# ComputationalPhysiology/oasisx

Measured on AMD Instinct MI355X. Metric: time-steps/sec, 3D Taylor-Green 128^3 P2-P1 (with pressure-CG SpMV GB/s in roofline), higher is better.
Workload: dtype f64

## Files before the change

### include/oasisx_hip.h

```cpp
#ifndef OASISX_HIP_H
#define OASISX_HIP_H

#include <stddef.h>
#include <stdint.h>

#ifdef __cplusplus
extern "C" {
#endif

#define OX_KV 2
#define OX_ROW_BLOCK_WAVES 8
#define OX_ROW_BLOCK_LDS (134 * 1024)
#define OX_SLICE 64

#define OX_CONVERGED_RTOL 2
#define OX_CONVERGED_ATOL 3
#define OX_CONVERGED_ITS 4
#define OX_DIVERGED_ITS (-3)
#define OX_DIVERGED_DTOL (-4)
#define OX_DIVERGED_BREAKDOWN (-5)
#define OX_DIVERGED_NANORINF (-9)

#define OX_KSP_CG 1
#define OX_KSP_BCGS 2
// ... 154 lines not shown
int ox_synchronize(void *stream);

int ox_version(void);
const char *ox_last_error(void);
int ox_sell_kv(void);
int ox_device_info(int *n_cu, char *name, int name_len);

int ox_spmv(const ox_sell *A, const double *x, double *y, int ncomp, const ox_dist *dist,
            void *stream);

int ox_sell_compress_cols(const ox_sell *A, uint16_t *cols16, int32_t *cbase, int64_t *n_compressed,
                          void *stream);

int ox_spmv_multi(int v2s, int gdim, const ox_sell *A, const double *x, const double *base, double scale,
                  double *y, const ox_dist *dist, void *stream);
int ox_assemble_rect(int family, int row_degree, int col_degree, const ox_cells *cells, const ox_adj *adj,
                     const uint8_t *adj_pos, int pw, const ox_sell *A, void *stream);

int ox_axpby(int64_t n, double a, const double *x, double b, const double *y, double *z,
             void *stream);
int ox_dot(int64_t n_rows, int ncomp, const double *x, const double *y, double *out_host,
           const ox_dist *dist, void *stream);

int ox_set_bc(double *b, const int32_t *dofs, const double *g, int64_t n, int ncomp, int comp,
              void *stream);

int ox_scatter_add(double *b, const int32_t *rows, const double *y, int64_t n, int ncomp, int comp,
                   double scale, void *stream);

int ox_zero_rows(const ox_sell *A, const int32_t *rows, int64_t n, double diag, void *stream);
int ox_zero_rows_au(const ox_sell *A, const int32_t *rows, int64_t n, double diag, double *au,
                    const double *u1, int ncomp, void *stream);
int ox_zero_rows_cols(const ox_sell *A, const uint8_t *is_bc, double diag, void *stream);

int ox_assemble_matrix(int kind, int degree, const ox_cells *cells, const int32_t *cell_dofs,
                       const ox_adj *adj, const uint8_t *adj_pos, int pw, const ox_sell *A,
                       int n_bins, const int64_t *bin_ptr_host, const int32_t *bin_slices,
                       const int32_t *bin_width_host, void *stream);
int ox_assemble_weights(int degree, const ox_cells *cells, const ox_adj *adj, int64_t n_rows,
                        double *w, void *stream);
int ox_assemble_load_vector(const ox_cells *cells, const ox_adj *adj, int64_t n_rows, int n_d, int n_q,
                            const double *wphi, const double *fq, double *b, void *stream);

int ox_assemble_first(int degree, const ox_cells *cells, const int32_t *cell_dofs,
                      const ox_adj *adj, const uint8_t *adj_pos, int pw, const ox_sell *A,
                      const ox_sell *M, const ox_sell *K, const double *uab,
// ... 49 lines not shown

size_t ox_ksp_work_bytes(int64_t n_rows, int64_t n_cols, int ncomp, int ksp_type);
int ox_ksp_solve(int ksp_type, const ox_sell *A, const double *dinv, const double *b, double *x,
                 int ncomp, double rtol, double atol, int max_it, int nonzero_guess,
                 int check_every, int max_restarts, void *work, size_t work_bytes,
                 ox_ksp_result *result, const ox_dist *dist, void *stream);
int ox_ksp_solve_ax0(int ksp_type, const ox_sell *A, const double *dinv, const double *b, double *x,
                     int ncomp, double rtol, double atol, int max_it, int nonzero_guess,
                     int check_every, int max_restarts, void *work, size_t work_bytes,
                     ox_ksp_result *result, const ox_dist *dist, void *stream, const double *ax0);
int ox_ksp_solve_dc(int ksp_type, const ox_sell *A, const double *dinv, const double *b, double *x,
                    int ncomp, double rtol, double atol, int max_it, int nonzero_guess,
                    int check_every, int max_restarts, void *work, size_t work_bytes,
                    ox_ksp_result *result, const ox_dist *dist, void *stream, const double *ax0,
                    const uint8_t *dinv_code, const double *dinv_dict, int n_dinv_dict);
typedef struct {
  double rtol, atol, divtol;
  int32_t max_it, nonzero_guess, check_every, max_restarts;
  int32_t fold_blocks, run_ahead;
  const double *ax0;
  const uint8_t *dinv_code;
  const double *dinv_dict;
  int32_t n_dinv_dict;
  int32_t reserved;
} ox_ksp_options;
int ox_ksp_options_default(ox_ksp_options *opt);
int ox_ksp_solve_opt(int ksp_type, const ox_sell *A, const double *dinv, const double *b, double *x, int ncomp,
                     const ox_ksp_options *opt, void *work, size_t work_bytes, ox_ksp_result *result,
                     const ox_dist *dist, void *stream);
size_t ox_ksp_work_bytes_for(const ox_sell *A, int ncomp, int ksp_type);

int ox_dg1_grad_rhs(int u_degree, const ox_cells *cells, const int32_t *cell_dofs, const double *u, double *b,
                    void *stream);
int ox_dg1_mass(int inverse, const ox_cells *cells, int ncomp, const double *in, double *out, void *stream);

int ox_remove_mean(int64_t n, int64_t n_apply, double *x, const double *w, double wsum,
                   const ox_dist *dist, void *stream);

int ox_ksp_default_fold_blocks(void);
int ox_ksp_kernels_per_iteration(int ksp_type, const ox_sell *A, int ncomp, int check_every, int fold_blocks,
                                 int partitioned);
int ox_profile_begin(int max_records, int sample_every);
int ox_profile_end(void);
int ox_profile_get(int tag, long long key, long long *count, double *total_ms);

int ox_range_push(const char *name);
int ox_range_pop(void);
// ... 94 lines not shown
```

### oasisx_amd/_lib.py

```python
from __future__ import annotations

import ctypes as C
import os

_HERE = os.path.dirname(os.path.abspath(__file__))
LIB_PATH = os.environ.get("OX_LIB_PATH") or os.path.join(_HERE, "liboasisx_hip.so")

KSP_CG, KSP_BCGS, KSP_CG_SINGLE, KSP_BCGS_MERGED, KSP_CG_MERGED = 1, 2, 3, 4, 5
KSP_CG_MG = 6
MG_MAX_DEGREE = 8
ROW_BLOCK_WAVES, ROW_BLOCK_LDS = 8, 134 * 1024
CONVERGED_RTOL, CONVERGED_ATOL, CONVERGED_ITS = 2, 3, 4
DIVERGED_ITS, DIVERGED_DTOL, DIVERGED_BREAKDOWN, DIVERGED_NANORINF = -3, -4, -5, -9


class OasisxHipError(RuntimeError):
    pass


class ox_sell(C.Structure):
    _fields_ = [
        ("n_rows", C.c_int64),
        ("n_cols", C.c_int64),
        ("n_slices", C.c_int32),
# ... 144 lines not shown
        ("reason", C.c_int32 * 4),
        ("its", C.c_int32 * 4),
        ("rnorm", C.c_double * 4),
        ("bnorm", C.c_double * 4),
        ("resumed", C.c_int32 * 4),
    ]


class ox_ksp_options(C.Structure):
    _fields_ = [
        ("rtol", C.c_double),
        ("atol", C.c_double),
        ("divtol", C.c_double),
        ("max_it", C.c_int32),
        ("nonzero_guess", C.c_int32),
        ("check_every", C.c_int32),
        ("max_restarts", C.c_int32),
        ("fold_blocks", C.c_int32),
        ("run_ahead", C.c_int32),
        ("ax0", C.c_void_p),
        ("dinv_code", C.c_void_p),
        ("dinv_dict", C.c_void_p),
        ("n_dinv_dict", C.c_int32),
        ("reserved", C.c_int32),
    ]


_P = C.c_void_p
_I = C.c_int
_L = C.c_int64
_D = C.c_double

SIGNATURES = {
    "ox_version": (_I, []),
    "ox_last_error": (C.c_char_p, []),
    "ox_sell_kv": (_I, []),
    "ox_device_info": (_I, [C.POINTER(_I), C.c_char_p, _I]),
    "ox_mesh_create": (_I, [_P, _L, _P, _L, _I, _I, _I, C.POINTER(_P)]),
    "ox_mesh_view": (_I, [_P, C.POINTER(ox_mesh_info)]),
    "ox_mesh_destroy": (_I, [_P]),
    "ox_space_create": (_I, [_P, _I, _I, C.POINTER(_P)]),
    "ox_space_create_ordered": (_I, [_P, _I, _I, _I, C.POINTER(_P)]),
    "ox_mesh_create_sub": (_I, [_P, _L, _P, _L, _I, _I, C.POINTER(_D), C.POINTER(_D), _I, _I, _L, C.POINTER(_P)]),
    "ox_space_create_part": (_I, [_P, _I, _I, _P, _L, _I, _L, C.POINTER(_P)]),
    "ox_space_view": (_I, [_P, C.POINTER(ox_space_info)]),
    "ox_space_windows": (_I, [_P, C.POINTER(ox_window_info)]),
    "ox_space_windows_split": (_I, [_P, _I, C.POINTER(ox_window_info)]),
    "ox_space_destroy": (_I, [_P]),
    "ox_rect_create": (_I, [_P, _P, C.POINTER(_P)]),
    "ox_rect_view": (_I, [_P, C.POINTER(ox_rect_info)]),
    "ox_rect_destroy": (_I, [_P]),
    "ox_value_dictionary": (_I, [_P, _L, _I, _P, _P, C.POINTER(_I), _P]),
    "ox_pair_stream_size": (_I, [C.POINTER(ox_sell), _P, _P, C.POINTER(_L), _P]),
    "ox_pair_stream_fill": (_I, [C.POINTER(ox_sell), _P, _P, _P, _P, C.POINTER(_L), _P]),
    "ox_malloc": (_I, [C.c_size_t, C.POINTER(_P)]),
    "ox_free": (_I, [_P]),
    "ox_memset": (_I, [_P, _I, C.c_size_t, _P]),
    "ox_synchronize": (_I, [_P]),
    "ox_spmv": (_I, [C.POINTER(ox_sell), _P, _P, _I, _P, _P]),
    "ox_sell_compress_cols": (_I, [C.POINTER(ox_sell), _P, _P, C.POINTER(_L), _P]),
    "ox_spmv_multi": (_I, [_I, _I, C.POINTER(ox_sell), _P, _P, _D, _P, _P, _P]),
    "ox_assemble_rect": (_I, [_I, _I, _I, C.POINTER(ox_cells), C.POINTER(ox_adj), _P, _I, C.POINTER(ox_sell), _P]),
    "ox_axpby": (_I, [_L, _D, _P, _D, _P, _P, _P]),
    "ox_dot": (_I, [_L, _I, _P, _P, C.POINTER(_D), _P, _P]),
    "ox_set_bc": (_I, [_P, _P, _P, _L, _I, _I, _P]),
    "ox_scatter_add": (_I, [_P, _P, _P, _L, _I, _I, _D, _P]),
    "ox_zero_rows": (_I, [C.POINTER(ox_sell), _P, _L, _D, _P]),
    "ox_zero_rows_au": (_I, [C.POINTER(ox_sell), _P, _L, _D, _P, _P, _I, _P]),
    "ox_zero_rows_cols": (_I, [C.POINTER(ox_sell), _P, _D, _P]),
    "ox_assemble_matrix": (_I, [_I, _I, C.POINTER(ox_cells), _P, C.POINTER(ox_adj), _P, _I,
                                C.POINTER(ox_sell), _I, C.POINTER(_L), _P, C.POINTER(C.c_int32), _P]),
    "ox_assemble_weights": (_I, [_I, C.POINTER(ox_cells), C.POINTER(ox_adj), _L, _P, _P]),
    "ox_assemble_load_vector": (_I, [C.POINTER(ox_cells), C.POINTER(ox_adj), _L, _I, _I, _P, _P, _P, _P]),
    "ox_assemble_first": (_I, [_I, C.POINTER(ox_cells), _P, C.POINTER(ox_adj), _P, _I,
                               C.POINTER(ox_sell), C.POINTER(ox_sell), C.POINTER(ox_sell), _P, _P, _P, _P, _D,
                               _D, _I, C.POINTER(_L), _P, C.POINTER(C.c_int32), _P]),
    "ox_assemble_first_au": (_I, [_I, C.POINTER(ox_cells), _P, C.POINTER(ox_adj), _P, _I,
                                  C.POINTER(ox_sell), C.POINTER(ox_sell), C.POINTER(ox_sell), _P, _P, _P, _P, _D,
                                  _D, _I, C.POINTER(_L), _P, C.POINTER(C.c_int32), _P, _P]),
    "ox_assemble_matrix_blocks": (_I, [_I, _I, C.POINTER(ox_cells), _P, C.POINTER(ox_adj), _P, _I, C.POINTER(ox_sell), _I, _P,
                                       _L, _P]),
    "ox_assemble_first_blocks": (_I, [_I, C.POINTER(ox_cells), _P, C.POINTER(ox_adj), _P, _I,
                                      C.POINTER(ox_sell), C.POINTER(ox_sell), C.POINTER(ox_sell), _P, _P, _P, _P, _D,
                                      _D, _I, _P, _L, _P, _P]),
    "ox_eddy_viscosity": (_I, [_I, _I, C.POINTER(ox_cells), _P, _P, _D, _P, _P]),
    "ox_assemble_first_au_nut": (_I, [_I, C.POINTER(ox_cells), _P, C.POINTER(ox_adj), _P, _I,
                                      C.POINTER(ox_sell), C.POINTER(ox_sell), C.POINTER(ox_sell), _P, _P, _P, _P, _D,
# ... 123 lines not shown
```

### oasisx_amd/csrc/ox_ksp.hip

```cpp
#include "ox_kernels.h"
#include "ox_ksp_dev.h"
#include "ox_p2p.h"
#include <type_traits>

struct KspPart2 {
  const double *partial;
  int nparts, nv;
};

__device__ __forceinline__ void ksp_gather2(const double *__restrict__ partial, int nparts, int nv, const KspPart2 &B,
                                            double (&v)[OX_MAX_NV]) {
  ox_gather_partials(partial, nparts, nv, v);
  if (B.nv > 0) {
    double w[OX_MAX_NV];
    ox_gather_partials(B.partial, B.nparts, B.nv, w);
#pragma unroll
    for (int i = 0; i < OX_MAX_NV; ++i)
#pragma unroll
      for (int j = 0; j < OX_MAX_NV; ++j)
        if (j == i - nv && j < B.nv) v[i] = w[j];
  }
}


// ... 932 lines not shown
    if (ox_prof_on) ox_prof_stop(st);
    OX_LAUNCH_CHECK();
    return 0;
  }
  hipLaunchKernelGGL((k_ksp_reduce<PH>), dim3(1), dim3(ox_red_threads(nmax)), 0, st, partial, nparts, nv, B, sums);
  OX_LAUNCH_CHECK();
  nv += B.nv;
  if (ox_allreduce_impl(dist, sums, nv, st)) return -1;
  hipLaunchKernelGGL((k_ksp_logic<PH>), dim3(1), dim3(64), 0, st, S, sums, P);
  if (ox_prof_on) ox_prof_stop(st);
  OX_LAUNCH_CHECK();
  return 0;
}

__global__ __launch_bounds__(256) void k_extract_col(int64_t n, const double *__restrict__ src, int nc,
                                                     int c, double *__restrict__ dst) {
  const int64_t stride = (int64_t)gridDim.x * 256;
  for (int64_t i = (int64_t)blockIdx.x * 256 + threadIdx.x; i < n; i += stride) dst[i] = src[i * nc + c];
}
__global__ __launch_bounds__(256) void k_insert_col(int64_t n, const double *__restrict__ src, int nc,
                                                    int c, double *__restrict__ dst) {
  const int64_t stride = (int64_t)gridDim.x * 256;
  for (int64_t i = (int64_t)blockIdx.x * 256 + threadIdx.x; i < n; i += stride) dst[i * nc + c] = src[i];
}

struct KspVecs {
  double *x, *r, *z, *p, *q;
  double *rhat, *v, *s, *t;
  double *u, *w;
};

struct KspCtx {
  const ox_sell *A;
  const double *dinv;
  KspDinv D;
  KspState *S, *S2;
  double *sums, *partial, *partial2;
  const ox_dist *dist;
  hipStream_t st;
  int nb, nbs;
  int fold;
};

#define KSP_SYNC(PH, partial, nparts, nv)                                                       \
  do {                                                                                          \
    if (ksp_sync_point<PH>(C.S, partial, nparts, nv, C.sums, P, C.dist, C.st)) return -1;       \
// ... 350 lines not shown
      if (queue(1 - cur)) return -1;
      it += batch;
    }
    OX_HIP(hipEventSynchronize(g_state_ev[cur]));
    if (C.dist && ox_dist_status(C.dist)) return -1;
    if (g_state_host[1 + cur].done || !more) {
      OX_HIP(hipStreamSynchronize(C.st));
      if (!more && !g_state_host[1 + cur].done) {
        OX_HIP(hipMemcpyAsync(g_state_host, C.S, sizeof(KspState), hipMemcpyDeviceToHost, C.st));
        OX_HIP(hipStreamSynchronize(C.st));
        return 0;
      }
      g_state_host[0] = g_state_host[1 + cur];
      return 0;
    }
    cur = 1 - cur;
  }
}

template <int NC>
static int ksp_run(int ksp_type, const ox_sell *A, const double *dinv, const double *b, double *x,
                   const KspParams &P, int guess, int check_every, char *work,
                   ox_ksp_result *result, const ox_dist *dist, hipStream_t st, const double *ax0, const KspDinv &Dc,
                   int fold_blocks, int run_ahead) {
  const int64_t n = A->n_rows;
  const KspLayout L = ksp_layout(A->n_rows, A->n_cols, NC, ksp_type, ksp_grid_max(A));
  KspCtx C;
  C.A = A;
  C.dinv = dinv;
  C.D = Dc;
  C.S = reinterpret_cast<KspState *>(work + L.state);
  C.S2 = reinterpret_cast<KspState *>(work + L.state2);
  C.sums = reinterpret_cast<double *>(work + L.sums);
  C.partial = reinterpret_cast<double *>(work + L.partial);
  C.partial2 = reinterpret_cast<double *>(work + L.partial2);
  C.dist = dist;
  C.st = st;
  C.nb = ox_vec_blocks(2 * (n > 0 ? n : 1));
  C.nbs = ox_spmv_dist_nparts(A, dist, NC);
  C.fold = fold_blocks;
  double *vec[6];
  for (int i = 0; i < L.nvec; ++i) vec[i] = reinterpret_cast<double *>(work + L.vec0 + L.vec_stride * i);
  if (!g_state_host) OX_HIP(hipHostMalloc(&g_state_host, 3 * sizeof(KspState)));
  const bool cg = ksp_type == OX_KSP_CG, cgs = ksp_type == OX_KSP_CG_SINGLE, bm = ksp_type == OX_KSP_BCGS_MERGED;
  const bool cgm = ksp_type == OX_KSP_CG_MERGED;
  KspVecs V{};
  V.x = x;
// ... 8 lines not shown
    if (ox_spmv_dist(A, V.u, V.w, NC, OX_EPI_DOT, nullptr, nullptr, C.partial2, nullptr, dist, st)) return -1;
    if (ksp_sync_point<PH_CGS_INIT>(C.S, C.partial, C.nb, 3 * NC, C.sums, P, dist, st, KspPart2{C.partial2, C.nbs, NC}))
      return -1;
  } else if (cg || cgm) {
    V.r = vec[0], V.p = vec[1], V.q = vec[2];
    if (guess && !ax0) {
      if (ox_spmv_dist(A, x, V.q, NC, OX_EPI_NONE, nullptr, nullptr, nullptr, nullptr, dist, st)) return -1;
    }
    hipLaunchKernelGGL((k_cg_init<NC>), dim3(C.nb), dim3(256), 0, st, n, b, x, (guess && ax0) ? ax0 : V.q, dinv, V.r,
                       V.p, guess, C.partial);
    OX_LAUNCH_CHECK();
    KSP_SYNC(PH_CG_INIT, C.partial, C.nb, 3 * NC);
  } else {
    V.r = vec[0], V.rhat = vec[1], V.p = vec[2], V.v = vec[3], V.s = vec[4], V.t = vec[5];
    if (guess && !ax0) {
      if (ox_spmv_dist(A, x, V.t, NC, OX_EPI_NONE, nullptr, nullptr, nullptr, nullptr, dist, st)) return -1;
    }
    hipLaunchKernelGGL((k_bcgs_init<NC>), dim3(C.nb), dim3(256), 0, st, n, b, x, (guess && ax0) ? ax0 : V.t, dinv, V.r,
                       V.rhat, V.p, V.v, guess, C.partial);
    OX_LAUNCH_CHECK();
    KSP_SYNC(PH_BCGS_INIT, C.partial, C.nb, 2 * NC);
  }
  bool bm_first = true;
  auto iterate = [&](auto nc_tag, const KspVecs &W, const KspParams &Q) -> int {
    constexpr int N_ = decltype(nc_tag)::value;
    const bool first = bm_first;
    bm_first = false;
    return cgs ? cgs_iterations<N_>(C, W, Q, check_every)
           : cgm ? cgm_iterations<N_>(C, W, Q, check_every, first)
               : (cg ? cg_iterations<N_>(C, W, Q, check_every)
                     : (bm ? bcgsm_iterations<N_>(C, W, Q, check_every, first) : bcgs_iterations<N_>(C, W, Q, check_every, first)));
  };
  auto batch_of = [&](int every) { return every > 8 ? 8 : every; };
  int it = 0;
  bool tail_done = false;
  for (;;) {
    tail_done = false;
    if (NC == 1 && run_ahead) {
      const int bsz = batch_of(check_every);
      auto it1 = [&](int count) -> int {
        const bool first = bm_first;
        bm_first = false;
        return cgs ? cgs_iterations<1>(C, V, P, count)
               : cgm ? cgm_iterations<1>(C, V, P, count, first)
                   : (cg ? cg_iterations<1>(C, V, P, count)
                         : (bm ? bcgsm_iterations<1>(C, V, P, count, first) : bcgs_iterations<1>(C, V, P, count, first)));
      };
      if (ksp_run_ahead(C, it1, bsz, it, P.max_it)) return -1;
    }
    for (; !(NC == 1 && run_ahead) && it <= P.max_it; it += check_every) {
      if (iterate(std::integral_constant<int, NC>{}, V, P)) return -1;
      if (ksp_read_state(C)) return -1;
      if (g_state_host->done) break;
      if (NC > 1) {
        int live = -1, nlive = 0;
        for (int c = 0; c < NC; ++c)
          if (g_state_host->active[c]) live = c, ++nlive;
        if (nlive == 1) {
          double *cv[8];
          for (int i = 0; i < 8; ++i) cv[i] = reinterpret_cast<double *>(work + L.narrow0 + L.narrow_stride * i);
          KspVecs W{};
          double *src[8] = {V.x, V.r, V.z, V.p, V.q, V.rhat, V.v, nullptr};
          double **dst[8] = {&W.x, &W.r, &W.z, &W.p, &W.q, &W.rhat, &W.v, nullptr};
          if (cg) src[2] = nullptr;
          if (cgs) {
            src[2] = V.u, dst[2] = &W.u;
            src[4] = V.s, dst[4] = &W.s;
            src[5] = V.w, dst[5] = &W.w;
            src[6] = nullptr;
          }
          for (int i = 0; i < 7; ++i) {
            *dst[i] = cv[i];
            if (!src[i]) continue;
            hipLaunchKernelGGL(k_extract_col, dim3(C.nb), dim3(256), 0, st, n, src[i], NC, live, cv[i]);
            OX_LAUNCH_CHECK();
          }
          if (!cgs) {
            W.s = cv[2];
            W.t = cv[4];
          }
          KspParams P1 = P;
          P1.nc = 1;
          P1.c0 = live;
          if (run_ahead) {
            const int bsz = batch_of(check_every);
            auto it1 = [&](int count) -> int {
              return cgs ? cgs_iterations<1>(C, W, P1, count)
                         : (cg ? cg_iterations<1>(C, W, P1, count)
                               : (bm ? bcgsm_iterations<1>(C, W, P1, count, false) : bcgs_iterations<1>(C, W, P1, count, false)));
            };
            it += check_every;
            if (ksp_run_ahead(C, it1, bsz, it, P.max_it)) return -1;
          } else {
            for (it += check_every; it <= P.max_it; it += check_every) {
              if (iterate(std::integral_constant<int, 1>{}, W, P1)) return -1;
              if (ksp_read_state(C)) return -1;
              if (g_state_host->done) break;
// ... 188 lines not shown
                               void *work, size_t work_bytes, ox_ksp_result *result, void *stream) {
  if (!mg || !A || !b || !x || !work || !result || !opt) OX_FAIL("ox_ksp_solve_mg: null argument");
  return mgcg_solve(mg, A, b, x, opt, work, work_bytes, result, nullptr, ox_stream(stream));
}

extern "C" int ox_ksp_solve_mg_dist(const ox_mg *mg, const ox_sell *A, const double *b, double *x, const ox_ksp_options *opt,
                                    void *work, size_t work_bytes, ox_ksp_result *result, const ox_dist *dist,
                                    void *stream) {
  if (!A || !b || !x || !work || !result || !opt || !dist) OX_FAIL("ox_ksp_solve_mg_dist: null argument");
  if (!mg && A->n_rows > 0) OX_FAIL("ox_ksp_solve_mg_dist: no hierarchy for %lld owned rows", (long long)A->n_rows);
  return mgcg_solve(mg, A, b, x, opt, work, work_bytes, result, dist, ox_stream(stream));
}

extern "C" int ox_ksp_options_default(ox_ksp_options *o) {
  if (!o) OX_FAIL("ox_ksp_options_default: null argument");
  memset(o, 0, sizeof(*o));
  o->rtol = 1e-5;
  o->atol = 1e-50;
  o->divtol = 1e4;
  o->max_it = 10000;
  o->check_every = 1;
  o->fold_blocks = -1;
  o->run_ahead = -1;
  return 0;
}

extern "C" int ox_ksp_default_fold_blocks(void) { return ksp_fold_blocks_default(); }

extern "C" int ox_ksp_kernels_per_iteration(int ksp_type, const ox_sell *A, int ncomp, int check_every, int fold_blocks,
                                            int partitioned) {
  if (!A) return -1;
  if (ksp_type == OX_KSP_CG_MERGED && ncomp > 1) ksp_type = OX_KSP_CG;
  const bool one = ncomp == 1 && !partitioned && A->n_rows >= 2 && ksp_fold_blocks_of(fold_blocks) > 0;
  const int batch = check_every > 8 ? 8 : (check_every < 1 ? 1 : check_every);
  switch (ksp_type) {
    case OX_KSP_CG: {
      if (!one) return 5;
      return ox_spmv_dist_nparts(A, nullptr, 1) >= OX_PRERED_MIN ? 4 : 3;
    }
    case OX_KSP_CG_MERGED:
      return (one && (batch & 1) == 0 && ox_spmv_dist_nparts(A, nullptr, 1) <= 10 * OX_FOLD_T) ? 2 : 3;
    case OX_KSP_CG_SINGLE: return 3;
    case OX_KSP_BCGS: return 8;
    case OX_KSP_BCGS_MERGED: return 6;
    default: return -1;
  }
// ... 9 lines not shown
  if (ksp_type == OX_KSP_CG_MERGED && ncomp > 1) ksp_type = OX_KSP_CG;
  if (ncomp < 1 || ncomp > OX_MAXC) OX_FAIL("ox_ksp_solve: ncomp=%d out of range", ncomp);
  if (work_bytes < ox_ksp_work_bytes_for(A, ncomp, ksp_type))
    OX_FAIL("ox_ksp_solve: workspace too small (%zu < %zu)", work_bytes, ox_ksp_work_bytes_for(A, ncomp, ksp_type));
  if (opt->dinv_code && (!opt->dinv_dict || opt->n_dinv_dict < 1 || opt->n_dinv_dict > 256))
    OX_FAIL("ox_ksp_solve: dinv dictionary of %d entries", opt->n_dinv_dict);
  if (!(opt->divtol > 0.0)) OX_FAIL("ox_ksp_solve: divtol=%g (must be positive; PETSc's default is 1e4)", opt->divtol);
  const int max_it = opt->max_it < 1 ? 1 : opt->max_it;
  const int check_every = opt->check_every < 1 ? 1 : opt->check_every;
  memset(result, 0, sizeof(*result));
  KspParams P{};
  P.rtol = opt->rtol;
  P.atol = opt->atol;
  P.dtol = opt->divtol;
  P.max_it = max_it;
  P.nc = ncomp;
  P.c0 = 0;
  P.nc_total = ncomp;
  P.max_restarts = opt->max_restarts < 0 ? 0 : opt->max_restarts;
  hipStream_t st = ox_stream(stream);
  char *w = static_cast<char *>(work);
  const KspDinv D{dinv, opt->dinv_code, opt->dinv_dict, opt->dinv_code ? opt->n_dinv_dict : 0};
  const int fold = ksp_fold_blocks_of(opt->fold_blocks), ahead = opt->run_ahead < 0 ? 1 : (opt->run_ahead ? 1 : 0);
  const int guess = opt->nonzero_guess;
  const double *ax0 = opt->ax0;
  switch (ncomp) {
    case 1: return ksp_run<1>(ksp_type, A, dinv, b, x, P, guess, check_every, w, result, dist, st, ax0, D, fold, ahead);
    case 2: return ksp_run<2>(ksp_type, A, dinv, b, x, P, guess, check_every, w, result, dist, st, ax0, D, fold, ahead);
    default: return ksp_run<3>(ksp_type, A, dinv, b, x, P, guess, check_every, w, result, dist, st, ax0, D, fold, ahead);
  }
}

extern "C" int ox_ksp_solve_dc(int ksp_type, const ox_sell *A, const double *dinv, const double *b,
                               double *x, int ncomp, double rtol, double atol, int max_it,
                               int nonzero_guess, int check_every, int max_restarts, void *work,
                               size_t work_bytes, ox_ksp_result *result, const ox_dist *dist, void *stream,
                               const double *ax0, const uint8_t *dinv_code, const double *dinv_dict, int n_dinv_dict) {
  ox_ksp_options o;
  ox_ksp_options_default(&o);
  o.rtol = rtol;
  o.atol = atol;
  o.max_it = max_it;
  o.nonzero_guess = nonzero_guess;
  o.check_every = check_every;
  o.max_restarts = max_restarts;
  o.ax0 = ax0;
  o.dinv_code = dinv_code;
  o.dinv_dict = dinv_dict;
  o.n_dinv_dict = n_dinv_dict;
  return ox_ksp_solve_opt(ksp_type, A, dinv, b, x, ncomp, &o, work, work_bytes, result, dist, stream);
}

// ... 17 lines not shown
```

### oasisx_amd/csrc/ox_spmv.hip

```cpp
#include "ox_common.h"
#include "ox_kernels.h"
#include <stdlib.h>
#include <type_traits>

thread_local char ox_err_buf[512] = "";

extern "C" int ox_version(void) { return 100; }
extern "C" const char *ox_last_error(void) { return ox_err_buf; }
extern "C" int ox_sell_kv(void) { return OX_KV; }

extern "C" int ox_device_info(int *n_cu, char *name, int name_len) {
  int dev = 0;
  OX_HIP(hipGetDevice(&dev));
  hipDeviceProp_t p;
  OX_HIP(hipGetDeviceProperties(&p, dev));
  if (n_cu) *n_cu = p.multiProcessorCount;
  if (name && name_len > 0) {
    strncpy(name, p.gcnArchName, name_len - 1);
    name[name_len - 1] = 0;
  }
  return 0;
}

template <int NC, int EPI, int VAR>
// ... 910 lines not shown
}

extern "C" int ox_dot(int64_t n_rows, int ncomp, const double *x, const double *y, double *out_host,
                      const ox_dist *dist, void *stream) {
  if (ncomp < 1 || ncomp > OX_MAXC) OX_FAIL("ox_dot: ncomp=%d", ncomp);
  if (ox_scratch_init()) return -1;
  hipStream_t st = ox_stream(stream);
  const int nblk = ox_vec_blocks(n_rows > 0 ? n_rows : 1);
  double *partial = g_scratch, *sums = g_scratch + OX_VEC_MAX_BLOCKS * 4;
  switch (ncomp) {
    case 1: hipLaunchKernelGGL(k_dot<1>, dim3(nblk), dim3(256), 0, st, n_rows, x, y, partial); break;
    case 2: hipLaunchKernelGGL(k_dot<2>, dim3(nblk), dim3(256), 0, st, n_rows, x, y, partial); break;
    default: hipLaunchKernelGGL(k_dot<3>, dim3(nblk), dim3(256), 0, st, n_rows, x, y, partial); break;
  }
  OX_LAUNCH_CHECK();
  if (ox_reduce_partials(partial, nblk, ncomp, sums, st)) return -1;
  if (dist && ox_allreduce_impl(dist, sums, ncomp, st)) return -1;
  OX_HIP(hipMemcpyAsync(g_scratch_host, sums, sizeof(double) * ncomp, hipMemcpyDeviceToHost, st));
  OX_HIP(hipStreamSynchronize(st));
  for (int c = 0; c < ncomp; ++c) out_host[c] = g_scratch_host[c];
  return 0;
}

__global__ __launch_bounds__(256) void k_wsum(int64_t n, const double *__restrict__ x,
                                              const double *__restrict__ w,
                                              double *__restrict__ partial) {
  __shared__ double red[4];
  double s[1] = {0.0};
  const int64_t stride = (int64_t)gridDim.x * 256;
  for (int64_t i = (int64_t)blockIdx.x * 256 + threadIdx.x; i < n; i += stride)
    s[0] += w ? w[i] * x[i] : x[i];
  ox_block_sum_256<1>(s, red);
  if (threadIdx.x == 0) partial[blockIdx.x] = s[0];
}
__global__ __launch_bounds__(256) void k_shift(int64_t n, double *x, const double *sum,
                                               double inv_wsum) {
  const double m = sum[0] * inv_wsum;
  const int64_t stride = (int64_t)gridDim.x * 256;
  for (int64_t i = (int64_t)blockIdx.x * 256 + threadIdx.x; i < n; i += stride) x[i] -= m;
}

extern "C" int ox_remove_mean(int64_t n, int64_t n_apply, double *x, const double *w, double wsum,
                              const ox_dist *dist, void *stream) {
  if (n_apply < n) n_apply = n;
  if (n_apply <= 0) return 0;
  if (ox_scratch_init()) return -1;
// ... 298 lines not shown
```

### oasisx_amd/fem.py

```python
from __future__ import annotations

import ctypes as C
import itertools

import numpy as np
import torch

from . import _lib
from .mesh import Mesh

KV = 2
SLICE = 64
default_scalar_type = np.float64


def local_edges(gdim: int):
    return [(1, 2), (0, 2), (0, 1)] if gdim == 2 else [(2, 3), (1, 3), (1, 2), (0, 3), (0, 2), (0, 1)]


import os as _os


def default_tile_bits(mesh: Mesh) -> int:
    env = _os.environ.get("OX_TILE_BITS")
# ... 1137 lines not shown
        self._V, self._i = V, i

    def collapse(self):
        n, dim = self._V.num_dofs, self._V.dim
        return self._V.scalar, (np.arange(n, dtype=np.int32) * dim + self._i)




class FieldStorage:

    def __init__(self, n: int, nc: int, device, n_alloc: int | None = None):
        self.n, self.nc = int(n), int(nc)
        self.n_alloc = int(n if n_alloc is None else n_alloc)
        self._dev = torch.zeros((self.n_alloc, self.nc), dtype=torch.float64, device=device)
        self._shared = self._dev.device.type == "cpu"
        self._host = self._dev.numpy()[: self.n] if self._shared else None
        self._out = False
        self.generation = 0

    def mark_written(self):
        self.generation += 1

    def host(self) -> np.ndarray:
        if self._shared:
            self.generation += 1
            return self._host
        if not self._out:
            if self._host is None:
                self._host = np.empty((self.n, self.nc))
            self._host[...] = self._dev[: self.n].cpu().numpy()
            self._out = True
        return self._host

    def _sync(self) -> torch.Tensor:
        if self._out:
            self._dev[: self.n].copy_(torch.from_numpy(self._host))
            self._out = False
            self.generation += 1
        return self._dev

    def dev(self) -> torch.Tensor:
        self._sync()
        self.generation += 1
        return self._dev

# ... 295 lines not shown
```

### oasisx_amd/fracstep.py

```python
from __future__ import annotations

import ctypes as C
import logging

import numpy as np
import torch

from . import _lib
from .fem import FieldStorage, Function, FunctionSpace, VectorFunctionSpace, cell_geometry
from .ksp import KSPSolver
from .la import MultiSellMatrix, SellMatrix

__all__ = ["FractionalStep_AB_CN"]


def _degree(element):
    if isinstance(element, FunctionSpace):
        return element.degree
    fam = str(element[0]).lower()
    if fam not in ("lagrange", "p", "cg"):
        raise ValueError(f"unsupported element family {element[0]!r}")
    return int(element[1])


# ... 128 lines not shown
        self._bcs_p = bcs_p
        with shared_marker_evaluations():
            for bc_i in self._bcs_u:
                for bc in bc_i:
                    bc.create_bc(Vi)
            for bcp in self._bcs_p:
                bcp.create_bcs(Vi, Q)
        if len(self._bcs_p) > 0:
            self._p_surf = [[bcp.rhs(i) for bcp in self._bcs_p] for i in range(gdim)]

        solver_options = {} if solver_options is None else solver_options
        self._solver_u = KSPSolver(mesh.comm, solver_options.get("tentative"), prefix="tentative_velocity")
        self._solver_p = KSPSolver(mesh.comm, solver_options.get("pressure"), prefix="pressure_correction")
        self._solver_c = KSPSolver(mesh.comm, solver_options.get("scalar"), prefix="velocity_update")
        self._rotational = bool(rotational)
        self._projector_p = None
        self._xi = 0.5 if rotational else None
        self._nu = 1.0 if rotational else None

        if options is None:
            options = {}
        self._low_memory = options.get("low_memory_version", True)
        self._options = dict(options)
        if body_force is None:
            body_force = (0.0,) * gdim
        from .function import Expression

        self._body_force = [f if (callable(f) or isinstance(f, (Function, Expression))) else float(f) for f in body_force]
        if len(self._body_force) != gdim:
            raise ValueError(f"body_force: {gdim} components expected")

        self._compile_and_allocate_forms()
        self._preassemble()
        self._nut = None
        if viscosity_model is not None:
            self._nut = torch.zeros(int(self._geom.shape[0]), dtype=torch.float64, device=dev)
            viscosity_model.bind(self)

        if self._rotational:
            from .function import Projector

            self._projector_p = Projector(_RotationalUpdate(self), Q, bcs=[],
                                          petsc_options=solver_options.get("scalar"), jit_options=jit_options)
        self._solver_p.setOperators(self._Ap)
        self._solver_p.setOptions(self._Ap)
        self._solver_c.setOperators(self._M)
# ... 207 lines not shown
            raise RuntimeError("effective_viscosity: the solver was built without a generalised-Newtonian law "
                               "(CarreauYasuda, Cross, PowerLaw)")
        return self.eddy_viscosity() + base

    @_phase
    def velocity_tentative_assemble(self):
        Vi, Q = self._Vi[0][0], self._Q
        if not self._low_memory:
            self._p_vdxi_Mat.mult(False, self._PS.ptr(), self._BFIRST.ptr(), 1.0, self._RHS1.ptr())
            return
        _lib.check(self._lib.ox_assemble_grad_vector(0, Vi.degree, Q.degree, C.byref(self._cells),
                                                     _lib.ptr(Q.cell_dofs), C.byref(self._adj_u), Vi.n_owned,
                                                     self._PS.ptr(), self._BFIRST.ptr(), 1.0, self._RHS1.ptr(),
                                                     _lib.current_stream()), "ox_assemble_grad_vector")

    @_phase
    def velocity_tentative_solve(self):
        lib, st = self._lib, _lib.current_stream()
        gdim = self._gdim
        for i in range(gdim):
            for bc in self._bcs_u[i]:
                bc.apply(self._rhs1[i].x)
        n = self._n_u * gdim
        _lib.check(lib.ox_axpby(n, 1.0, self._U.rptr(), 0.0, None, self._WRK.ptr(), st), "ox_axpby")
        ax0 = None
        if getattr(self, "_AU1_valid", False):
            self._AU1_valid = False
            same = getattr(self, "_u_is_u1", None) == (self._U.generation, self._U1.generation)
            if self._part is not None and getattr(self._comm, "size", 1) > 1:
                same = self._comm.allreduce(0.0 if same else 1.0, op="max") == 0.0
            if same:
                ax0 = self._B3
            elif not getattr(self, "_shortcut_note", False):
                self._shortcut_note = True
                logging.getLogger("oasisx").info(
                    "tentative solve: u was handed out writable since the last step (FieldStorage.dev() / ptr() / host()): "
                    "the A u1 product of assemble_first is not reused; read-only access goes through rdev() / rptr() / rhost()")
        self._u_is_u1 = None
        errors = np.asarray(self._solver_u.solve_block(self._RHS1, self._U, ax0=ax0), dtype=np.int32)
        _lib.check(lib.ox_axpby(n, 1.0, self._WRK.ptr(), -1.0, self._U.ptr(), self._WRK.ptr(), st), "ox_axpby")
        out = (C.c_double * 4)()
        _lib.check(lib.ox_dot(self._no_u, gdim, self._WRK.ptr(), self._WRK.ptr(), out, self._du, st), "ox_dot")
        diff = float(sum(np.sqrt(out[i]) for i in range(gdim)))
        return diff, errors

    @_phase
    def pressure_assemble(self, dt: float):
        Vi, Q = self._Vi[0][0], self._Q
        if not self._low_memory:
            self._divu_Mat.mult(True, self._U.ptr(), None, -1.0 / float(dt), self._B2.ptr())
        else:
            _lib.check(self._lib.ox_assemble_div_vector(Q.degree, Vi.degree, C.byref(self._cells),
                                                        _lib.ptr(Vi.cell_dofs), C.byref(self._adj_q), Q.n_owned,
                                                        self._U.ptr(), -1.0 / float(dt), self._B2.ptr(),
                                                        _lib.current_stream()), "ox_assemble_div_vector")
        for bcp in self._bcs_p:
            bcp.apply_homogeneous(self._b2.x)

    @_phase
    def pressure_solve(self, nu: float | None = None, rotational: bool = False):
        lib, st = self._lib, _lib.current_stream()
        logger = logging.getLogger("oasisx")
        nq, nqo = self._n_q, self._no_q
        if len(self._bcs_p) == 0:
            if "ksp_error_if_not_converged" not in self._solver_p._options:
# ... 70 lines not shown
        nq, n = self._n_q, self._n_u * self._gdim
        _lib.check(lib.ox_axpby(nq, 1.0, self._P.ptr(), 0.0, None, self._PS.ptr(), st), "ox_axpby")
        for bcu in self._bcs_u:
            for bc in bcu:
                bc.update_bc()
        for g in self._scalar_groups:
            for m in g.members:
                for bc in m.bcs:
                    bc.update_bc()
        self.assemble_first(dt, nu)
        while inner_it < max_iter and diff > max_error:
            inner_it += 1
            self.velocity_tentative_assemble()
            diff, errors = self.velocity_tentative_solve()
            assert (errors > 0).all(), f"tentative velocity solve failed: {errors}"
            self.pressure_assemble(dt)
            error_p = self.pressure_solve(nu=nu)
            assert int(error_p) > 0, f"pressure solve failed: {error_p}"
        errors_c = self.velocity_update(dt)
        self._last_errors = (errors, error_p, errors_c)
        if self._scalar_groups:
            reasons = self.scalar_solve()
            assert all(r > 0 for r in reasons.values()), f"scalar transport solve failed: {reasons}"
        _lib.check(lib.ox_axpby(n, 1.0, self._U1.ptr(), 0.0, None, self._U2.ptr(), st), "ox_axpby")
        _lib.check(lib.ox_axpby(n, 1.0, self._U.ptr(), 0.0, None, self._U1.ptr(), st), "ox_axpby")
        _lib.check(lib.ox_axpby(nq, 1.0, self._PS.ptr(), 0.0, None, self._P.ptr(), st), "ox_axpby")
        self._u_is_u1 = (self._U.generation, self._U1.generation)
        for d_ in (self._du, self._dq):
            if d_ is not None:
                _lib.check(lib.ox_dist_status(d_), "ox_dist_status (halo exchange / all-reduce of this step)")
        return diff

    @property
    def u(self):
        return self._sol_u

    def iteration_counts(self):
        its = {"tentative": self._solver_u.iterations, "pressure": self._solver_p.iterations,
               "update": self._solver_c.iterations}
        if self._scalar_groups:
            its["scalar_transport"] = {m.name: (g.ksp.iterations[j] if g.ksp.iterations else None)
                                       for g in self._scalar_groups for j, m in enumerate(g.members)}
        return its
```

### oasisx_amd/ksp.py

```python
from __future__ import annotations

import ctypes as C
import logging
import os
import typing

import torch

from . import _lib
from .fem import FieldStorage, Function
from .la import SellMatrix

__all__ = ["KSPSolver", "KSPConvergenceError"]


class KSPConvergenceError(RuntimeError):

    def __init__(self, prefix, reasons, its):
        self.reasons, self.iterations = list(reasons), list(its)
        names = {-3: "DIVERGED_ITS", -4: "DIVERGED_DTOL", -5: "DIVERGED_BREAKDOWN", -9: "DIVERGED_NANORINF"}
        what = ", ".join(f"{names.get(r, r)} after {i} iterations" for r, i in zip(self.reasons, self.iterations) if r <= 0)
        super().__init__(f"KSPSolver[{prefix}]: KSPSolve has not converged ({what})")


# ... 54 lines not shown
        return int(_lib.load().ox_guess_dim(self.handle))

    def __del__(self):
        h = getattr(self, "handle", None)
        if h is not None and h.value:
            try:
                _lib.load().ox_guess_destroy(h)
            except Exception:
                pass
            self.handle = None


class KSPSolver:
    def __init__(self, comm=None, petsc_options: typing.Optional[dict] = None, prefix="oasis_solver"):
        self._comm = comm
        self._prefix = prefix
        self._options: dict = {}
        self._A: SellMatrix | None = None
        self._dinv = None
        self._dinv_version = -1
        self._work = None
        self.last_result = None
        self.check_every = None
        self._every = {}
        self._env_fold = _env_int("OX_CG_FOLD_BLOCKS", -1)
        self._env_ahead = _env_int("OX_KSP_RUN_AHEAD", -1)
        self._mg = None
        self._mg_key = None
        self._guess = None
        self._guess_key = None
        self.updateOptions({} if petsc_options is None else petsc_options)

    def updateOptions(self, options: dict):
        self._options.update({str(k): v for k, v in options.items()})

    def _audit_options(self, nc: int = 1):
        log = logging.getLogger("oasisx")
        seen = self.__dict__.setdefault("_warned", set())

        def warn(key, msg, level=logging.WARNING):
            tag = (key, str(self._options.get(key)))
            if tag not in seen:
                seen.add(tag)
                log.log(level, "KSPSolver[%s]: %s", self._prefix, msg)

        o = self._options
# ... 275 lines not shown
                nd = C.c_int(0)
                _lib.check(lib.ox_value_dictionary(_lib.ptr(self._dinv), A.pattern.n_rows, 1, _lib.ptr(code), _lib.ptr(vdict),
                                                   C.byref(nd), st), "ox_value_dictionary")
                if nd.value > 0:
                    self._dcode, self._ddict = code, vdict[: nd.value]
        need = lib.ox_ksp_work_bytes_for(A.ref(), nc, meth)
        if self._work is None or self._work.shape[0] < need:
            self._work = torch.empty(int(need), dtype=torch.uint8, device=dev)
        g = self._guess_for(nc)
        nonzero, ax0_ptr = self._guess_form(g, B, X, guess, ax0)
        res = _lib.ox_ksp_result()
        key = (nc, meth)
        if key not in self._every:
            self._every[key] = self._interval_for(nc, meth)
        every = self.check_every or self._every[key]
        restarts = int(self._options.get("ksp_bcgs_restarts", 5 if direct else 0))
        dcode = getattr(self, "_dcode", None)
        opt = _lib.ox_ksp_options()
        _lib.check(lib.ox_ksp_options_default(C.byref(opt)), "ox_ksp_options_default")
        opt.rtol, opt.atol, opt.max_it = rtol, atol, max_it
        opt.divtol = float(self._options.get("ksp_divtol", 1e4))
        opt.nonzero_guess, opt.check_every, opt.max_restarts = int(nonzero), int(every), restarts
        opt.fold_blocks, opt.run_ahead = self._fold_blocks(), self._run_ahead()
        opt.ax0 = ax0_ptr
        if dcode is not None:
            opt.dinv_code, opt.dinv_dict = _lib.ptr(dcode), _lib.ptr(self._ddict)
            opt.n_dinv_dict = int(self._ddict.shape[0])
        _lib.check(lib.ox_ksp_solve_opt(meth, A.ref(), _lib.ptr(self._dinv), B.ptr(), X.ptr(), nc, C.byref(opt),
                                        _lib.ptr(self._work), int(self._work.shape[0]), C.byref(res), A.pattern.dist, st),
                   "ox_ksp_solve")
        if A.pattern.dist is not None:
            _lib.check(lib.ox_halo_forward(A.pattern.dist, X.ptr(), nc, st), "ox_halo_forward")
        self.last_result = res
        reasons = [int(res.reason[c]) for c in range(nc)]
        self._guess_update(g, X, reasons)
        if direct:
            reasons = [_lib.CONVERGED_ITS if r > 0 else r for r in reasons]
        if _truthy(self._options.get("ksp_error_if_not_converged", False)) and any(r <= 0 for r in reasons):
            raise KSPConvergenceError(self._prefix, reasons, [int(res.its[c]) for c in range(nc)])
        return reasons

    def _solve_gamg(self, B: FieldStorage, X: FieldStorage, ax0):
        lib = _lib.load()
        A = self._A
        self._audit_options(1)
        mg = self._hierarchy()
# ... 59 lines not shown
```

Before: 12.20.

## Add step shortcuts: fused diff-norm, buffer swap, batched column extract, mirrored KSP state

Several independent shortcuts are added to each time step. When u still equals u1, the tentative-velocity convergence norm comes from a fused difference-norm kernel on U1 and U, which removes the copy into a work buffer and the subtract pass. The U2 update is now a pointer exchange with U1 instead of a device copy. In the multi-component KSP loop, the column extractions run in one batched kernel, and the solver state is read through a mirrored host buffer plus an event sync. Together these aim to cut memory passes, kernel launches and host round trips, at the cost of extra code paths guarded by a default-on option.

Result: no change. 12.25, median of 3 (+0.4%).

```diff
diff --git a/include/oasisx_hip.h b/include/oasisx_hip.h
--- a/include/oasisx_hip.h
+++ b/include/oasisx_hip.h
@@ -200,6 +200,9 @@
 int ox_dot(int64_t n_rows, int ncomp, const double *x, const double *y, double *out_host,
            const ox_dist *dist, void *stream);
 
+int ox_diff_norm2(int64_t n_rows, int ncomp, const double *a, const double *b, double *out_host,
+                  const ox_dist *dist, void *stream);
+
 int ox_set_bc(double *b, const int32_t *dofs, const double *g, int64_t n, int ncomp, int comp,
               void *stream);
 
@@ -295,7 +298,7 @@
   const uint8_t *dinv_code;
   const double *dinv_dict;
   int32_t n_dinv_dict;
-  int32_t reserved;
+  int32_t step_shortcuts;
 } ox_ksp_options;
 int ox_ksp_options_default(ox_ksp_options *opt);
 int ox_ksp_solve_opt(int ksp_type, const ox_sell *A, const double *dinv, const double *b, double *x, int ncomp,
diff --git a/oasisx_amd/_lib.py b/oasisx_amd/_lib.py
--- a/oasisx_amd/_lib.py
+++ b/oasisx_amd/_lib.py
@@ -190,7 +190,7 @@
         ("dinv_code", C.c_void_p),
         ("dinv_dict", C.c_void_p),
         ("n_dinv_dict", C.c_int32),
-        ("reserved", C.c_int32),
+        ("step_shortcuts", C.c_int32),
     ]
 
 
@@ -231,6 +231,7 @@
     "ox_assemble_rect": (_I, [_I, _I, _I, C.POINTER(ox_cells), C.POINTER(ox_adj), _P, _I, C.POINTER(ox_sell), _P]),
     "ox_axpby": (_I, [_L, _D, _P, _D, _P, _P, _P]),
     "ox_dot": (_I, [_L, _I, _P, _P, C.POINTER(_D), _P, _P]),
+    "ox_diff_norm2": (_I, [_L, _I, _P, _P, C.POINTER(_D), _P, _P]),
     "ox_set_bc": (_I, [_P, _P, _P, _L, _I, _I, _P]),
     "ox_scatter_add": (_I, [_P, _P, _P, _L, _I, _I, _D, _P]),
     "ox_zero_rows": (_I, [C.POINTER(ox_sell), _P, _L, _D, _P]),
diff --git a/oasisx_amd/csrc/ox_ksp.hip b/oasisx_amd/csrc/ox_ksp.hip
--- a/oasisx_amd/csrc/ox_ksp.hip
+++ b/oasisx_amd/csrc/ox_ksp.hip
@@ -978,6 +978,25 @@
                                                     int c, double *__restrict__ dst) {
   const int64_t stride = (int64_t)gridDim.x * 256;
   for (int64_t i = (int64_t)blockIdx.x * 256 + threadIdx.x; i < n; i += stride) dst[i * nc + c] = src[i];
+}
+
+#define OX_EXTRACT_MAX 6
+struct KspExtract {
+  const double *src[OX_EXTRACT_MAX];
+  double *dst[OX_EXTRACT_MAX];
+  int count;
+};
+__global__ __launch_bounds__(256) void k_extract_cols(int64_t n, int nc, int c, KspExtract X) {
+  const int64_t stride = (int64_t)gridDim.x * 256;
+  for (int64_t i = (int64_t)blockIdx.x * 256 + threadIdx.x; i < n; i += stride) {
+    double v[OX_EXTRACT_MAX];
+#pragma unroll
+    for (int k = 0; k < OX_EXTRACT_MAX; ++k)
+      if (k < X.count) v[k] = X.src[k][i * nc + c];
+#pragma unroll
+    for (int k = 0; k < OX_EXTRACT_MAX; ++k)
+      if (k < X.count) X.dst[k][i] = v[k];
+  }
 }
 
 struct KspVecs {
@@ -1374,7 +1393,7 @@
 static int ksp_run(int ksp_type, const ox_sell *A, const double *dinv, const double *b, double *x,
                    const KspParams &P, int guess, int check_every, char *work,
                    ox_ksp_result *result, const ox_dist *dist, hipStream_t st, const double *ax0, const KspDinv &Dc,
-                   int fold_blocks, int run_ahead) {
+                   int fold_blocks, int run_ahead, int shortcuts) {
   const int64_t n = A->n_rows;
   const KspLayout L = ksp_layout(A->n_rows, A->n_cols, NC, ksp_type, ksp_grid_max(A));
   KspCtx C;
@@ -1429,6 +1448,7 @@
     KSP_SYNC(PH_BCGS_INIT, C.partial, C.nb, 2 * NC);
   }
   bool bm_first = true;
+  const bool sc = shortcuts && !dist && NC > 1;
   auto iterate = [&](auto nc_tag, const KspVecs &W, const KspParams &Q) -> int {
     constexpr int N_ = decltype(nc_tag)::value;
     const bool first = bm_first;
@@ -1456,8 +1476,20 @@
       if (ksp_run_ahead(C, it1, bsz, it, P.max_it)) return -1;
     }
     for (; !(NC == 1 && run_ahead) && it <= P.max_it; it += check_every) {
-      if (iterate(std::integral_constant<int, NC>{}, V, P)) return -1;
-      if (ksp_read_state(C)) return -1;
+      if (sc) {
+        if (!g_state_ev[0]) OX_HIP(hipEventCreateWithFlags(&g_state_ev[0], hipEventDisableTiming));
+        g_state_host[1].done = 0;
+        g_batch_mirror = g_state_host + 1;
+        const int rc = iterate(std::integral_constant<int, NC>{}, V, P);
+        g_batch_mirror = nullptr;
+        if (rc) return -1;
+        OX_HIP(hipEventRecord(g_state_ev[0], st));
+        OX_HIP(hipEventSynchronize(g_state_ev[0]));
+        g_state_host[0] = g_state_host[1];
+      } else {
+        if (iterate(std::integral_constant<int, NC>{}, V, P)) return -1;
+        if (ksp_read_state(C)) return -1;
+      }
       if (g_state_host->done) break;
       if (NC > 1) {
         int live = -1, nlive = 0;
@@ -1476,10 +1508,25 @@
             src[5] = V.w, dst[5] = &W.w;
             src[6] = nullptr;
           }
+          if (sc) {
+            if (cg) src[4] = nullptr;
+            if (bm) src[6] = nullptr;
+            if (cgs) src[2] = nullptr;
+          }
+          KspExtract X{};
           for (int i = 0; i < 7; ++i) {
             *dst[i] = cv[i];
             if (!src[i]) continue;
+            if (sc) {
+              X.src[X.count] = src[i], X.dst[X.count] = cv[i];
+              ++X.count;
+              continue;
+            }
             hipLaunchKernelGGL(k_extract_col, dim3(C.nb), dim3(256), 0, st, n, src[i], NC, live, cv[i]);
+            OX_LAUNCH_CHECK();
+          }
+          if (sc) {
+            hipLaunchKernelGGL(k_extract_cols, dim3(C.nb), dim3(256), 0, st, n, NC, live, X);
             OX_LAUNCH_CHECK();
           }
           if (!cgs) {
@@ -1714,6 +1761,7 @@
   o->check_every = 1;
   o->fold_blocks = -1;
   o->run_ahead = -1;
+  o->step_shortcuts = 1;
   return 0;
 }
 
@@ -1769,12 +1817,12 @@
   char *w = static_cast<char *>(work);
   const KspDinv D{dinv, opt->dinv_code, opt->dinv_dict, opt->dinv_code ? opt->n_dinv_dict : 0};
   const int fold = ksp_fold_blocks_of(opt->fold_blocks), ahead = opt->run_ahead < 0 ? 1 : (opt->run_ahead ? 1 : 0);
-  const int guess = opt->nonzero_guess;
+  const int guess = opt->nonzero_guess, sc = opt->step_shortcuts ? 1 : 0;
   const double *ax0 = opt->ax0;
   switch (ncomp) {
-    case 1: return ksp_run<1>(ksp_type, A, dinv, b, x, P, guess, check_every, w, result, dist, st, ax0, D, fold, ahead);
-    case 2: return ksp_run<2>(ksp_type, A, dinv, b, x, P, guess, check_every, w, result, dist, st, ax0, D, fold, ahead);
-    default: return ksp_run<3>(ksp_type, A, dinv, b, x, P, guess, check_every, w, result, dist, st, ax0, D, fold, ahead);
+    case 1: return ksp_run<1>(ksp_type, A, dinv, b, x, P, guess, check_every, w, result, dist, st, ax0, D, fold, ahead, sc);
+    case 2: return ksp_run<2>(ksp_type, A, dinv, b, x, P, guess, check_every, w, result, dist, st, ax0, D, fold, ahead, sc);
+    default: return ksp_run<3>(ksp_type, A, dinv, b, x, P, guess, check_every, w, result, dist, st, ax0, D, fold, ahead, sc);
   }
 }
 
diff --git a/oasisx_amd/csrc/ox_spmv.hip b/oasisx_amd/csrc/ox_spmv.hip
--- a/oasisx_amd/csrc/ox_spmv.hip
+++ b/oasisx_amd/csrc/ox_spmv.hip
@@ -956,6 +956,50 @@
   return 0;
 }
 
+template <int NC>
+__global__ __launch_bounds__(256) void k_diff_dot(int64_t n_rows, const double *__restrict__ a,
+                                                  const double *__restrict__ b, double *__restrict__ partial) {
+  __shared__ double red[4 * NC];
+  double s[NC];
+#pragma unroll
+  for (int c = 0; c < NC; ++c) s[c] = 0.0;
+  const int64_t stride = (int64_t)gridDim.x * 256;
+  for (int64_t r = (int64_t)blockIdx.x * 256 + threadIdx.x; r < n_rows; r += stride) {
+#pragma unroll
+    for (int c = 0; c < NC; ++c) {
+      const double d = a[r * NC + c] - b[r * NC + c];
+      s[c] = fma(d, d, s[c]);
+    }
+  }
+  ox_block_sum_256<NC>(s, red);
+  if (threadIdx.x == 0) {
+#pragma unroll
+    for (int c = 0; c < NC; ++c) partial[(size_t)blockIdx.x * NC + c] = s[c];
+  }
+}
+
+extern "C" int ox_diff_norm2(int64_t n_rows, int ncomp, const double *a, const double *b, double *out_host,
+                             const ox_dist *dist, void *stream) {
+  if (ncomp < 1 || ncomp > 3) OX_FAIL("ox_diff_norm2: ncomp=%d", ncomp);
+  if (!a || !b || !out_host) OX_FAIL("ox_diff_norm2: null argument");
+  if (ox_scratch_init()) return -1;
+  hipStream_t st = ox_stream(stream);
+  const int nblk = ox_vec_blocks(n_rows > 0 ? n_rows : 1);
+  double *partial = g_scratch, *sums = g_scratch + OX_VEC_MAX_BLOCKS * 4;
+  switch (ncomp) {
+    case 1: hipLaunchKernelGGL(k_diff_dot<1>, dim3(nblk), dim3(256), 0, st, n_rows, a, b, partial); break;
+    case 2: hipLaunchKernelGGL(k_diff_dot<2>, dim3(nblk), dim3(256), 0, st, n_rows, a, b, partial); break;
+    default: hipLaunchKernelGGL(k_diff_dot<3>, dim3(nblk), dim3(256), 0, st, n_rows, a, b, partial); break;
+  }
+  OX_LAUNCH_CHECK();
+  if (ox_reduce_partials(partial, nblk, ncomp, sums, st)) return -1;
+  if (dist && ox_allreduce_impl(dist, sums, ncomp, st)) return -1;
+  OX_HIP(hipMemcpyAsync(g_scratch_host, sums, sizeof(double) * ncomp, hipMemcpyDeviceToHost, st));
+  OX_HIP(hipStreamSynchronize(st));
+  for (int c = 0; c < ncomp; ++c) out_host[c] = g_scratch_host[c];
+  return 0;
+}
+
 __global__ __launch_bounds__(256) void k_wsum(int64_t n, const double *__restrict__ x,
                                               const double *__restrict__ w,
                                               double *__restrict__ partial) {
diff --git a/oasisx_amd/fem.py b/oasisx_amd/fem.py
--- a/oasisx_amd/fem.py
+++ b/oasisx_amd/fem.py
@@ -1183,6 +1183,16 @@
     def mark_written(self):
         self.generation += 1
 
+    def exchange(self, other: "FieldStorage"):
+        if (self.n, self.nc, self.n_alloc) != (other.n, other.nc, other.n_alloc):
+            raise ValueError("FieldStorage.exchange: the two blocks differ in shape")
+        self._sync()
+        other._sync()
+        self._dev, other._dev = other._dev, self._dev
+        self._host, other._host = other._host, self._host
+        self.generation += 1
+        other.generation += 1
+
     def host(self) -> np.ndarray:
         if self._shared:
             self.generation += 1
diff --git a/oasisx_amd/fracstep.py b/oasisx_amd/fracstep.py
--- a/oasisx_amd/fracstep.py
+++ b/oasisx_amd/fracstep.py
@@ -174,6 +174,9 @@
             options = {}
         self._low_memory = options.get("low_memory_version", True)
         self._options = dict(options)
+        self._shortcuts = bool(options.get("step_shortcuts", True))
+        for ksp_ in (self._solver_u, self._solver_p, self._solver_c):
+            ksp_.step_shortcuts = self._shortcuts
         if body_force is None:
             body_force = (0.0,) * gdim
         from .function import Expression
@@ -427,25 +430,33 @@
             for bc in self._bcs_u[i]:
                 bc.apply(self._rhs1[i].x)
         n = self._n_u * gdim
-        _lib.check(lib.ox_axpby(n, 1.0, self._U.rptr(), 0.0, None, self._WRK.ptr(), st), "ox_axpby")
+        au1 = getattr(self, "_AU1_valid", False)
+        self._AU1_valid = False
         ax0 = None
-        if getattr(self, "_AU1_valid", False):
-            self._AU1_valid = False
+        same = False
+        if au1 or self._shortcuts:
             same = getattr(self, "_u_is_u1", None) == (self._U.generation, self._U1.generation)
             if self._part is not None and getattr(self._comm, "size", 1) > 1:
                 same = self._comm.allreduce(0.0 if same else 1.0, op="max") == 0.0
-            if same:
+            if same and au1:
                 ax0 = self._B3
-            elif not getattr(self, "_shortcut_note", False):
+            elif au1 and not getattr(self, "_shortcut_note", False):
                 self._shortcut_note = True
                 logging.getLogger("oasisx").info(
                     "tentative solve: u was handed out writable since the last step (FieldStorage.dev() / ptr() / host()): "
                     "the A u1 product of assemble_first is not reused; read-only access goes through rdev() / rptr() / rhost()")
+        old_is_u1 = same and self._shortcuts
+        if not old_is_u1:
+            _lib.check(lib.ox_axpby(n, 1.0, self._U.rptr(), 0.0, None, self._WRK.ptr(), st), "ox_axpby")
         self._u_is_u1 = None
         errors = np.asarray(self._solver_u.solve_block(self._RHS1, self._U, ax0=ax0), dtype=np.int32)
-        _lib.check(lib.ox_axpby(n, 1.0, self._WRK.ptr(), -1.0, self._U.ptr(), self._WRK.ptr(), st), "ox_axpby")
         out = (C.c_double * 4)()
-        _lib.check(lib.ox_dot(self._no_u, gdim, self._WRK.ptr(), self._WRK.ptr(), out, self._du, st), "ox_dot")
+        if old_is_u1:
+            _lib.check(lib.ox_diff_norm2(self._no_u, gdim, self._U1.rptr(), self._U.rptr(), out, self._du, st),
+                       "ox_diff_norm2")
+        else:
+            _lib.check(lib.ox_axpby(n, 1.0, self._WRK.ptr(), -1.0, self._U.ptr(), self._WRK.ptr(), st), "ox_axpby")
+            _lib.check(lib.ox_dot(self._no_u, gdim, self._WRK.ptr(), self._WRK.ptr(), out, self._du, st), "ox_dot")
         diff = float(sum(np.sqrt(out[i]) for i in range(gdim)))
         return diff, errors
 
@@ -562,7 +573,10 @@
         if self._scalar_groups:
             reasons = self.scalar_solve()
             assert all(r > 0 for r in reasons.values()), f"scalar transport solve failed: {reasons}"
-        _lib.check(lib.ox_axpby(n, 1.0, self._U1.ptr(), 0.0, None, self._U2.ptr(), st), "ox_axpby")
+        if self._shortcuts:
+            self._U2.exchange(self._U1)
+        else:
+            _lib.check(lib.ox_axpby(n, 1.0, self._U1.ptr(), 0.0, None, self._U2.ptr(), st), "ox_axpby")
         _lib.check(lib.ox_axpby(n, 1.0, self._U.ptr(), 0.0, None, self._U1.ptr(), st), "ox_axpby")
         _lib.check(lib.ox_axpby(nq, 1.0, self._PS.ptr(), 0.0, None, self._P.ptr(), st), "ox_axpby")
         self._u_is_u1 = (self._U.generation, self._U1.generation)
diff --git a/oasisx_amd/ksp.py b/oasisx_amd/ksp.py
--- a/oasisx_amd/ksp.py
+++ b/oasisx_amd/ksp.py
@@ -100,6 +100,7 @@
         self._work = None
         self.last_result = None
         self.check_every = None
+        self.step_shortcuts = True
         self._every = {}
         self._env_fold = _env_int("OX_CG_FOLD_BLOCKS", -1)
         self._env_ahead = _env_int("OX_KSP_RUN_AHEAD", -1)
@@ -421,6 +422,7 @@
         opt.divtol = float(self._options.get("ksp_divtol", 1e4))
         opt.nonzero_guess, opt.check_every, opt.max_restarts = int(nonzero), int(every), restarts
         opt.fold_blocks, opt.run_ahead = self._fold_blocks(), self._run_ahead()
+        opt.step_shortcuts = int(bool(self.step_shortcuts))
         opt.ax0 = ax0_ptr
         if dcode is not None:
             opt.dinv_code, opt.dinv_dict = _lib.ptr(dcode), _lib.ptr(self._ddict)
```
